# Shadylukin/Neumann

Measured on AMD Instinct MI355X. Metric: queries/sec, brute-force SIMILAR TOP-K (recall@K = 1.0 vs CPU oracle), higher is better.
Workload: dtype f32

## Files before the change

neumann_amd/csrc/nmn_api.hip:

```cpp
#include <algorithm>
#include <atomic>
#include <chrono>
#include <thread>
#include <cmath>
#include <cstdio>
#include <cstdlib>
#include <cstring>
#include <mutex>
#include <new>
#include <string>
#include <unordered_map>
#include <vector>

#include "nmn_index.h"

using namespace nmn;

namespace nmn {
float synth_value_host(uint64_t seed, uint64_t row, uint32_t col);
}

static thread_local std::string g_last_error;

static nmn_status fail_hip(hipError_t e, const char* what) {
// ... 177 lines not shown
static nmn_status ws_alloc_core(nmn_index* idx, Workspace* w);
static nmn_status ws_get(nmn_index* idx, hipStream_t stream, uint32_t nq, uint32_t k, Workspace** out) {
    Workspace* w = nullptr;
    auto it = idx->ws.find(stream);
    if (it != idx->ws.end()) w = it->second;
    uint32_t nqc = std::min(pass_queries(idx, nq), idx->ws_nq_limit);
    uint32_t cand_cap = std::max<uint32_t>(std::min<uint32_t>(idx->cand_cap, NMN_MAX_TOP_K), std::min<uint32_t>(k, NMN_MAX_TOP_K));
    if (w && w->nq_cap >= nqc && w->cand_cap >= cand_cap) {
        *out = w;
        return NMN_OK;
    }
    if (w) {
        HIP_TRY(hipStreamSynchronize(stream));
        nqc = std::max(nqc, w->nq_cap);
        cand_cap = std::max(cand_cap, w->cand_cap);
        if (w->allocated && w->cand_cap >= cand_cap) {
            Workspace* wn = new (std::nothrow) Workspace();
            if (!wn) return fail_arg(NMN_ERR_OUT_OF_MEMORY, "workspace alloc");
            wn->stream = stream;
            wn->nq_cap = nqc;
            wn->cand_cap = cand_cap;
            const nmn_status st = ws_alloc_core(idx, wn);
            if (st == NMN_OK) {
                wn->allocated = true;
                idx->ws.erase(stream);
                ws_free(w);
                idx->ws[stream] = wn;
                *out = wn;
                return NMN_OK;
            }
            ws_free(wn);
            if (st != NMN_ERR_OUT_OF_MEMORY) return st;
            idx->ws_nq_limit = std::min(idx->ws_nq_limit, w->nq_cap);
            *out = w;
            return NMN_OK;
        }
        idx->ws.erase(stream);
        ws_free(w);
    }
    w = new (std::nothrow) Workspace();
    if (!w) return fail_arg(NMN_ERR_OUT_OF_MEMORY, "workspace alloc");
    w->stream = stream;
    w->nq_cap = nqc;
    w->cand_cap = cand_cap;
    idx->ws[stream] = w;
    *out = w;
    return NMN_OK;
}

constexpr uint64_t kCrowdMinRows = 1ull << 18;
constexpr uint64_t kCrowdPool = 8ull << 20;

static void ws_release_core(Workspace* w) {
    void** ptrs[] = {(void**)&w->scores, (void**)&w->tmax, (void**)&w->wmax, (void**)&w->tsample, (void**)&w->skip_key,
                     (void**)&w->k_extra, (void**)&w->qpad, (void**)&w->qi8, (void**)&w->qinfo, (void**)&w->qinfo_f32, (void**)&w->qstate,
                     (void**)&w->cand_rows, (void**)&w->cand_scores, (void**)&w->split_sg, (void**)&w->split_ctr, (void**)&w->final_ticket, (void**)&w->done_ctr, (void**)&w->run_slots, (void**)&w->run_bound, (void**)&w->h_counts2, (void**)&w->crowd_ctr,
                     (void**)&w->crowd_rows, (void**)&w->crowd_scores, (void**)&w->fb_hist, (void**)&w->fb_list, (void**)&w->fb_count,
                     (void**)&w->fb_sync};
    for (void** p : ptrs) {
        if (*p) (void)hipFree(*p);
        *p = nullptr;
    }
    w->crowd_cap = 0;
    for (auto& e : w->ev) {
        if (e) (void)hipEventDestroy(e);
        e = nullptr;
    }
    for (auto& e : w->hist) {
        if (e) (void)hipEventDestroy(e);
        e = nullptr;
    }
    w->hist_head = w->hist_read = 0;
    w->allocated = false;
}

static nmn_status ws_alloc_core(nmn_index* idx, Workspace* w) {
    w->ld = idx->ld;
    w->score_stride = idx->cap_pad;
    w->n_tiles_cap = (uint32_t)(idx->cap_pad / kTileRows);
    const size_t nq = w->nq_cap;
    {
        static const long test_max_nq = [] { const char* e = getenv("NMN_WS_TEST_MAX_NQ"); return e ? atol(e) : 0l; }();
        if (test_max_nq > 0 && (long)nq > test_max_nq) return fail_hip(hipErrorOutOfMemory, "workspace (NMN_WS_TEST_MAX_NQ)");
    }
    HIP_TRY(hipMalloc(reinterpret_cast<void**>(&w->scores), std::max<size_t>(nq * w->score_stride, 64) * 4));
    w->tmax_stride = ((uint64_t)w->n_tiles_cap + 3) & ~3ull;
    HIP_TRY(hipMalloc(reinterpret_cast<void**>(&w->tmax), std::max<size_t>(nq * w->tmax_stride, 4) * 4));
    HIP_TRY(hipMalloc(reinterpret_cast<void**>(&w->wmax), nq * kMaxScanWaves * 4));
    w->n_sample_cap = (w->n_tiles_cap + kSampleStep - 1) / kSampleStep + 4;
    HIP_TRY(hipMalloc(reinterpret_cast<void**>(&w->tsample), nq * w->n_sample_cap * 4));
    HIP_TRY(hipMalloc(reinterpret_cast<void**>(&w->skip_key), nq * 4));
    HIP_TRY(hipMalloc(reinterpret_cast<void**>(&w->k_extra), 4));
    HIP_TRY(hipMalloc(reinterpret_cast<void**>(&w->qpad), nq * w->ld * sizeof(float)));
    HIP_TRY(hipMalloc(reinterpret_cast<void**>(&w->qi8), nq * w->ld * 2));
    HIP_TRY(hipMalloc(reinterpret_cast<void**>(&w->qinfo), nq * sizeof(QInfo)));
    HIP_TRY(hipMalloc(reinterpret_cast<void**>(&w->qinfo_f32), nq * sizeof(QInfo)));
    HIP_TRY(hipMalloc(reinterpret_cast<void**>(&w->qstate), nq * sizeof(QState)));
    HIP_TRY(hipMalloc(reinterpret_cast<void**>(&w->cand_rows), nq * w->cand_cap * sizeof(uint32_t)));
    HIP_TRY(hipMalloc(reinterpret_cast<void**>(&w->cand_scores), nq * w->cand_cap * sizeof(float)));
    {
        const size_t nqs = std::min<size_t>(nq, 4);
        HIP_TRY(hipMalloc(reinterpret_cast<void**>(&w->split_sg), nqs * 1024 * 4));
        HIP_TRY(hipMemset(w->split_sg, 0, nqs * 1024 * 4));
        HIP_TRY(hipMalloc(reinterpret_cast<void**>(&w->split_ctr), nqs * 16));
        HIP_TRY(hipMemset(w->split_ctr, 0, nqs * 16));
    }
    HIP_TRY(hipMalloc(reinterpret_cast<void**>(&w->final_ticket), nq * 4));
    HIP_TRY(hipMalloc(reinterpret_cast<void**>(&w->done_ctr), 4));
    HIP_TRY(hipMemset(w->done_ctr, 0, 4));
    HIP_TRY(hipMalloc(reinterpret_cast<void**>(&w->run_slots), nq * 1024 * 4));
    HIP_TRY(hipMalloc(reinterpret_cast<void**>(&w->run_bound), ((nq + 127) & ~(size_t)127) * 4 + 512));
    HIP_TRY(hipMemset(w->run_bound, 0, ((nq + 127) & ~(size_t)127) * 4 + 512));
    HIP_TRY(hipMemset(w->final_ticket, 0, nq * 4));
    HIP_TRY(hipMalloc(reinterpret_cast<void**>(&w->h_counts2), 2 * sizeof(unsigned long long)));
    if (idx->cap_pad >= kCrowdMinRows) {
        w->crowd_cap = (uint32_t)std::min<uint64_t>(std::max<uint64_t>(kCrowdPool, (uint64_t)nq << 17),
                                                    std::max<uint64_t>(idx->cap_pad, (uint64_t)nq * (idx->cap_pad / 8)));
        HIP_TRY(hipMalloc(reinterpret_cast<void**>(&w->crowd_ctr), (3 + (size_t)kCrowdMaxGrid) * nq * 4));
        HIP_TRY(hipMemset(w->crowd_ctr, 0, (3 + (size_t)kCrowdMaxGrid) * nq * 4));
        HIP_TRY(hipMalloc(reinterpret_cast<void**>(&w->crowd_rows), (size_t)w->crowd_cap * 4));
        HIP_TRY(hipMalloc(reinterpret_cast<void**>(&w->crowd_scores), (size_t)w->crowd_cap * 4));
        HIP_TRY(hipMalloc(reinterpret_cast<void**>(&w->fb_hist), (6 * 2048 + 2) * 4));
        HIP_TRY(hipMalloc(reinterpret_cast<void**>(&w->fb_list), nq * (size_t)NMN_MAX_TOP_K * 8));
        HIP_TRY(hipMalloc(reinterpret_cast<void**>(&w->fb_count), nq * 4));
        HIP_TRY(hipMalloc(reinterpret_cast<void**>(&w->fb_sync), 16));
        HIP_TRY(hipMemset(w->fb_sync, 0, 16));
    }
    for (auto& e : w->ev) HIP_TRY(hipEventCreate(&e));
    return NMN_OK;
}

static nmn_status ws_alloc(nmn_index* idx, Workspace* w) {
    if (w->allocated) return NMN_OK;
    for (;;) {
        const nmn_status st = ws_alloc_core(idx, w);
        if (st == NMN_OK) break;
        const std::string keep = g_last_error;
        ws_release_core(w);
        g_last_error = keep;
        if (st != NMN_ERR_OUT_OF_MEMORY || w->nq_cap <= 1) return st;
        w->nq_cap = std::max<uint32_t>(1, w->nq_cap / 4);
// ... 666 lines not shown
            sp.i8_scale = idx->q8_scale;
            sp.i8_vv = idx->q8_vv;
            sp.i8_cos = idx->q8_cos;
            sp.qi8 = w->qi8;
            sp.norms = idx->norms;
            sp.inv_norms = idx->inv_norms;
            sp.qpad = w->qpad;
            sp.qinfo = w->qinfo;
            sp.mask = mask_dev;
            sp.qmasks = qmasks_dev ? qmasks_dev + qa : nullptr;
            sp.scores = w->scores;
            sp.tmax = w->tmax;
            sp.wmax = w->wmax;
            sp.tmax_stride = w->tmax_stride;
            sp.wmax_stride = kMaxScanWaves;
            sp.n_rows = n_rows;
            sp.nql = nqc;
            sp.ld = idx->ld;
            sp.n_tiles = n_tiles;
            sp.nq = nqc;
            static const uint32_t wave_target = [] {
                const char* e = getenv("NMN_SCAN_WAVES");
                long v = e ? atol(e) : (long)kMaxScanWaves;
                return (uint32_t)std::min<long>(std::max<long>(v, 256), (long)kMaxScanWaves);
            }();
            sp.tiles_per_wave = std::max<uint32_t>(1, (n_tiles + wave_target - 1) / wave_target);
            static const bool waves_pinned = getenv("NMN_SCAN_WAVES") != nullptr;
            static const uint32_t small_waves = [] {
                const char* e = getenv("NMN_SCAN_WAVES_SMALL");
                const long v = e ? atol(e) : 768;
                return v <= 0 ? 0u : (uint32_t)std::min<long>(std::max<long>(v, 256), (long)kMaxScanWaves);
            }();
            {
                const uint64_t sweep_bytes = (uint64_t)n_rows * idx->ld * w->last_elem_bytes;
                if (!waves_pinned && small_waves && !use_mfma && !mask_dev && sweep_bytes >= (128ull << 20) && sweep_bytes < (2ull << 30))
                    sp.tiles_per_wave = std::max<uint32_t>(1, (n_tiles + small_waves - 1) / small_waves);
            }
            static const uint32_t mfma_wgs = [] {
                const char* e = getenv("NMN_MFMA_WGS");
                long v = e ? atol(e) : 1024;
                return (uint32_t)std::min<long>(std::max<long>(v, 64), (long)kMaxScanWaves);
            }();
            if (use_mfma) sp.tiles_per_wave = std::max<uint32_t>(1, (n_tiles + mfma_wgs - 1) / mfma_wgs);
            auto launch_batch_sweep = [&](const ScanParams& x) -> hipError_t { return launch_scan_mfma(x, stream); };
            static const bool no_ring = getenv("NMN_NO_RING") != nullptr;
            const bool use_ring = !no_ring && !use_mfma && !use_i8 && !use_half && nqc == 1 && !mask_dev && !qmasks_dev && n_tiles >= 4096u &&
                                  metric != NMN_METRIC_SPARSE_COSINE_F64 && scan_ring_supported(idx->ld, idx->dim, (int)metric);
            static const uint32_t ring_wgs = [] {
                const char* e = getenv("NMN_RING_WGS");
                long v = e ? atol(e) : (long)kMaxScanWaves;
                return (uint32_t)std::min<long>(std::max<long>(v, 64), (long)kMaxScanWaves);
            }();
            if (use_ring) sp.tiles_per_wave = std::max<uint32_t>(1, (n_tiles + ring_wgs - 1) / ring_wgs);
            sp.metric = (int)metric;
            sp.strided = (!use_mfma && mask_dev) ? 1u : 0u;
            static const bool no_walk = getenv("NMN_NO_WALK") != nullptr;
            sp.walk = (sp.strided && !no_walk) ? 1u : 0u;
            sp.tile_step = 1;
            sp.skip_key = nullptr;
            static const uint32_t sample_step = [] {
                const char* e = getenv("NMN_SAMPLE_STEP");
                const long v = e ? atol(e) : 0;
                return (v == 64 || v == 128 || v == 256) ? (uint32_t)v : kSampleStep;
            }();
            static const bool sample_behind = getenv("NMN_SAMPLE_AHEAD_OF_CHAIN") == nullptr;
            const uint32_t n_sample = (n_tiles + sample_step - 1) / sample_step;
            static const uint32_t run_dbg = [] { const char* e = getenv("NMN_RUN_BOUND_DEBUG"); return e ? (uint32_t)atol(e) : 0u; }();
            const bool sample = use_mfma && (!run_bound || (run_dbg & 1u)) && n_sample >= 4u * k && n_sample >= 1024u && !no_sample();
            if (run_bound) {
                sp.run_slots = w->run_slots;
                sp.run_bound = w->run_bound;
                sp.run_S = run_S;
                sp.run_dbg = run_dbg;
            }
            auto sampling_pass = [&]() -> nmn_status {
                ScanParams ss = sp;
                ss.run_S = 0;
                ss.tile_step = sample_step;
                ss.n_tiles = n_sample;
                ss.tiles_per_wave = std::max<uint32_t>(1, (n_sample + 255) / 256);
                ss.tmax = w->tsample;
                ss.tmax_stride = w->n_sample_cap;
                static const bool reread_env = getenv("NMN_SAMPLE_REREAD") != nullptr;
                const bool reread = reread_env || use_i8;
                if (!reread) {
                    ss.tmax_main = w->tmax;
                    ss.tmax_main_stride = w->tmax_stride;
                }
                HIP_TRY(launch_batch_sweep(ss));
                HIP_TRY(launch_sample_bound(w->tsample, w->n_sample_cap, n_sample, w->qinfo, nqc, k, w->skip_key, stream));
                sp.skip_key = w->skip_key;
                sp.skip_sampled = reread ? 0u : sample_step;
                return NMN_OK;
            };
            if (sample && !sample_behind) {
                st = sampling_pass();
                if (st != NMN_OK) return st;
            }
            static const bool no_chain = getenv("NMN_NO_SWEEP_CHAIN") != nullptr;
            const bool chain = !no_chain && (uint64_t)n_rows * idx->ld * w->last_elem_bytes >= (2ull << 30);
            if (chain && idx->sweep_seq && idx->sweep_stream != stream)
                HIP_TRY(hipStreamWaitEvent(stream, idx->sweep_ev[(idx->sweep_seq - 1) & 3u], 0));
            if (w->timed && qa == 0 && !nested) {
                hipEvent_t& h = w->hist[2 * (w->hist_head % Workspace::kTimingHistory)];
                if (!h) HIP_TRY(hipEventCreate(&h));
                HIP_TRY(hipEventRecord(h, stream));
            }
            if (sample && sample_behind) {
                st = sampling_pass();
                if (st != NMN_OK) return st;
            }
            static const bool no_refine = getenv("NMN_NO_REFINE") != nullptr;
            const uint32_t mfma_blocks = use_mfma ? (n_tiles + sp.tiles_per_wave - 1) / sp.tiles_per_wave : 0;
            static const uint32_t n_cu = [] {
                int dev = 0, n = 256;
                if (hipGetDevice(&dev) != hipSuccess || hipDeviceGetAttribute(&n, hipDeviceAttributeMultiprocessorCount, dev) != hipSuccess || n <= 0) n = 256;
                return (uint32_t)n;
            }();
            const uint32_t first_blocks = mfma_blocks >= 3u * n_cu ? (n_cu & ~7u) : 0u;
            static const uint32_t refine_min_nq = [] {
                const char* e = getenv("NMN_REFINE_MIN_NQ");
                return e ? (uint32_t)atol(e) : 65u;
            }();
            const uint32_t refine_from = ((use_i8 || mfma_f32) && !getenv("NMN_REFINE_MIN_NQ")) ? 3u : refine_min_nq;
            const bool refine = use_mfma && sample && nqc >= refine_from && !no_refine && first_blocks >= 64 && (uint64_t)first_blocks * sp.tiles_per_wave >= 4ull * k;
            if (qa == 0) {
                w->last_sweep_kind = use_mfma ? (use_i8 ? NMN_SWEEP_MFMA_I8 : use_half ? NMN_SWEEP_MFMA_BF16 : NMN_SWEEP_MFMA_F32)
                                              : use_i8 ? NMN_SWEEP_VALU_I8 : use_ring ? NMN_SWEEP_RING_F32 : use_half ? NMN_SWEEP_VALU_BF16 : NMN_SWEEP_VALU_F32;
                w->last_sweep_launches = (sample ? 2u : 0u) + (refine ? 3u : 1u);
            }
            if (refine) {
                ScanParams sa = sp;
                sa.bx_base = 0;
                sa.bx_count = first_blocks;
                HIP_TRY(launch_batch_sweep(sa));
                HIP_TRY(launch_sample_bound(w->tmax, w->tmax_stride, first_blocks * sp.tiles_per_wave, w->qinfo, nqc, k, w->skip_key, stream, 1));
                ScanParams sb = sp;
                sb.bx_base = first_blocks;
                sb.bx_count = 0;
                HIP_TRY(launch_batch_sweep(sb));
            } else {
                HIP_TRY(use_mfma ? launch_batch_sweep(sp) : use_i8 ? launch_scan_i8(sp, stream) : use_ring ? launch_scan_ring(sp, stream) : launch_scan(sp, stream));
            }
            if (w->timed && qa == 0 && !nested) {
                hipEvent_t& h = w->hist[2 * (w->hist_head % Workspace::kTimingHistory) + 1];
                if (!h) HIP_TRY(hipEventCreate(&h));
                HIP_TRY(hipEventRecord(h, stream));
                w->hist_head++;
                w->scan_ev_in_hist = true;
            }
            if (chain) {
                hipEvent_t& ce = idx->sweep_ev[idx->sweep_seq & 3u];
                if (!ce) HIP_TRY(hipEventCreateWithFlags(&ce, hipEventDisableTiming));
// ... 848 lines not shown
    *calls_per_s = (double)calls.load() / dt;
    if (merged_batches) *merged_batches = b1 - b0;
    if (merged_calls) *merged_calls = r1 - r0;
    if (mismatches) *mismatches = bad.load();
    return NMN_OK;
}

extern "C" nmn_status nmn_index_coalesce_stats(nmn_index* idx, uint64_t* batches, uint64_t* requests) {
    if (!idx) return fail_arg(NMN_ERR_INVALID_ARGUMENT, "null index");
    std::lock_guard<std::mutex> g(idx->mu);
    if (batches) *batches = idx->coalesced_batches;
    if (requests) *requests = idx->coalesced_requests;
    return NMN_OK;
}

extern "C" nmn_status nmn_index_search(nmn_index* idx, const float* queries, uint32_t nq, uint32_t k,
                                       nmn_metric metric, const uint64_t* mask, uint64_t* out_rows,
                                       float* out_scores, uint32_t* out_counts, nmn_search_stats* stats) {
    const nmn_status st = index_search_hostio(idx, queries, nq, k, (int)metric, mask, false, out_rows, out_scores, out_counts, stats);
    if (st == NMN_OK && stats && mask && stats->rows_scanned && idx->dim) {
        const uint64_t n = stats->rows_scanned, eb = stats->bytes_scanned / (n * idx->dim);
        uint64_t kept = 0;
        for (uint64_t wd = 0; wd < n / 64; wd++) kept += (uint64_t)__builtin_popcountll(mask[wd]);
        if (n % 64) kept += (uint64_t)__builtin_popcountll(mask[n / 64] & ((1ull << (n % 64)) - 1));
        stats->rows_scanned = kept;
        stats->bytes_scanned = kept * idx->dim * eb;
    }
    return st;
}

extern "C" nmn_status nmn_index_search_dmask(nmn_index* idx, const float* queries, uint32_t nq, uint32_t k,
                                             nmn_metric metric, const uint64_t* mask_dev, uint64_t* out_rows,
                                             float* out_scores, uint32_t* out_counts, nmn_search_stats* stats) {
    return index_search_hostio(idx, queries, nq, k, (int)metric, mask_dev, true, out_rows, out_scores, out_counts, stats);
}

extern "C" nmn_status nmn_index_search_dmask_hint(nmn_index* idx, const float* queries, uint32_t nq, uint32_t k,
                                                  nmn_metric metric, const uint64_t* mask_dev, uint64_t mask_rows,
                                                  uint64_t* out_rows, float* out_scores, uint32_t* out_counts,
                                                  nmn_search_stats* stats) {
    return index_search_hostio(idx, queries, nq, k, (int)metric, mask_dev, true, out_rows, out_scores, out_counts, stats,
                               mask_rows);
}

extern "C" nmn_status nmn_index_read_probe(nmn_index* idx, uint32_t reps, double* gbps_out) {
    if (!idx || !gbps_out) return fail_arg(NMN_ERR_INVALID_ARGUMENT, "null argument");
    *gbps_out = 0.0;
    if (idx->rows == 0) return NMN_OK;
    HIP_TRY(hipSetDevice(idx->device));
    std::unique_lock<std::mutex> lk(idx->mu);
    IdleGuard idle(idx, lk);
    hipStream_t s = idx->host_stream;
    float* sink = nullptr;
    HIP_TRY(hipMalloc(reinterpret_cast<void**>(&sink), 4));
    hipEvent_t a = nullptr, b = nullptr;
    hipError_t e = hipEventCreate(&a);
    if (e == hipSuccess) e = hipEventCreate(&b);
    float best = 0.f;
    const uint64_t n_tiles = idx->rows / kTileRows;
    const bool ring = n_tiles >= 4096u && scan_ring_supported(idx->ld, idx->dim, NMN_METRIC_DOT_PRODUCT) && !getenv("NMN_NO_RING");
    const uint32_t ring_tpw = (uint32_t)std::max<uint64_t>(1, (n_tiles + kMaxScanWaves - 1) / kMaxScanWaves);
    uint64_t probe_rows = ring ? n_tiles * kTileRows : idx->rows;
    auto probe = [&]() { return ring ? launch_ring_probe(idx->corpus, idx->rows, idx->ld, ring_tpw, s) : launch_read_probe(idx->corpus, idx->rows, idx->ld, sink, s); };
    if (e == hipSuccess) e = probe();
    for (uint32_t i = 0; i < std::max(reps, 1u) && e == hipSuccess; i++) {
        e = hipEventRecord(a, s);
        if (e == hipSuccess) e = probe();
        if (e == hipSuccess) e = hipEventRecord(b, s);
        if (e == hipSuccess) e = hipEventSynchronize(b);
        float ms = 0.f;
        if (e == hipSuccess) e = hipEventElapsedTime(&ms, a, b);
        if (e == hipSuccess && ms > 0.f && (best == 0.f || ms < best)) best = ms;
    }
    if (a) (void)hipEventDestroy(a);
    if (b) (void)hipEventDestroy(b);
    (void)hipFree(sink);
    if (e != hipSuccess) return fail_hip(e, "nmn_index_read_probe");
    if (best > 0.f) *gbps_out = (double)probe_rows * idx->ld * 4.0 / (best * 1e-3) / 1e9;
    return NMN_OK;
}

extern "C" nmn_status nmn_index_score_rows(nmn_index* idx, const float* queries, uint32_t nq, nmn_metric metric,
                                           const uint64_t* local_rows, uint32_t n_rows, float* out_scores) {
    if (!idx || !queries || !local_rows || !out_scores) return fail_arg(NMN_ERR_INVALID_ARGUMENT, "null argument");
    if (nq == 0 || n_rows == 0) return NMN_OK;
    if (nq > NMN_MAX_QUERIES) return fail_arg(NMN_ERR_INVALID_ARGUMENT, "nq out of range");
    for (uint32_t i = 0; i < n_rows; i++)
        if (local_rows[i] >= idx->rows) return fail_arg(NMN_ERR_NOT_FOUND, "row out of range");
    HIP_TRY(hipSetDevice(idx->device));
    std::unique_lock<std::mutex> lk(idx->mu);
    IdleGuard idle(idx, lk);
    hipStream_t s = idx->host_stream;
    float *dq = nullptr, *dqpad = nullptr, *dout = nullptr;
    QInfo* dqi = nullptr;
    QState* dqs = nullptr;
    uint64_t* drows = nullptr;
    auto done = [&](nmn_status st) {
        for (void* p : {(void*)dq, (void*)dqpad, (void*)dout, (void*)dqi, (void*)dqs, (void*)drows})
            if (p) (void)hipFree(p);
        return st;
    };
    hipError_t e;
#define TRY2(x) if ((e = (x)) != hipSuccess) return done(fail_hip(e, #x))
    TRY2(hipMalloc(reinterpret_cast<void**>(&dq), (size_t)nq * idx->dim * 4));
    TRY2(hipMalloc(reinterpret_cast<void**>(&dqpad), (size_t)nq * idx->ld * 4));
    TRY2(hipMalloc(reinterpret_cast<void**>(&dout), (size_t)nq * n_rows * 4));
    TRY2(hipMalloc(reinterpret_cast<void**>(&dqi), (size_t)nq * sizeof(QInfo)));
    TRY2(hipMalloc(reinterpret_cast<void**>(&dqs), (size_t)nq * sizeof(QState)));
    TRY2(hipMalloc(reinterpret_cast<void**>(&drows), (size_t)n_rows * 8));
    TRY2(hipMemcpyAsync(dq, queries, (size_t)nq * idx->dim * 4, hipMemcpyHostToDevice, s));
    TRY2(hipMemcpyAsync(drows, local_rows, (size_t)n_rows * 8, hipMemcpyHostToDevice, s));
    TRY2(launch_qprep(dq, nq, idx->dim, idx->ld, (int)metric, idx->max_norm_bits, dqpad, dqi, dqs, 0, s));
    TRY2(launch_score_rows(idx->corpus, idx->norms, dqpad, dqi, drows, n_rows, nq, idx->ld, idx->dim, (int)metric,
                           dout, s));
    TRY2(hipMemcpyAsync(out_scores, dout, (size_t)nq * n_rows * 4, hipMemcpyDeviceToHost, s));
    TRY2(hipStreamSynchronize(s));
// ... 157 lines not shown
```

neumann_amd/csrc/nmn_index.h:

```cpp
#pragma once
#include <condition_variable>
#include <mutex>
#include <string>
#include <unordered_map>
#include <vector>

#include "nmn_internal.h"

using nmn::QInfo;
using nmn::QState;
using nmn::kDefaultCandCap;

struct Workspace {
    hipStream_t stream = nullptr;
    uint32_t nq_cap = 0;
    uint32_t cand_cap = 0;
    uint64_t score_stride = 0;
    uint32_t n_tiles_cap = 0;
    uint32_t ld = 0;
    uint32_t* scores = nullptr;
    uint32_t* tmax = nullptr;
    uint32_t* wmax = nullptr;
    uint32_t* tsample = nullptr;
    uint32_t* skip_key = nullptr;
    uint32_t* k_extra = nullptr;
    uint32_t* crowd_ctr = nullptr;
    uint32_t* crowd_rows = nullptr;
    float* crowd_scores = nullptr;
    uint32_t crowd_cap = 0;
    uint32_t* fb_hist = nullptr;
    unsigned long long* fb_list = nullptr;
    uint32_t* fb_count = nullptr;
    unsigned long long* fb_sync = nullptr;
    uint64_t n_sample_cap = 0;
    uint64_t tmax_stride = 0;
    float* qpad = nullptr;
    uint32_t* qi8 = nullptr;
    QInfo* qinfo = nullptr;
    QInfo* qinfo_f32 = nullptr;
    QState* qstate = nullptr;
    uint32_t* cand_rows = nullptr;
    float* cand_scores = nullptr;
    uint32_t* run_slots = nullptr;
    uint32_t* run_bound = nullptr;
    uint32_t* split_sg = nullptr;
    uint32_t* split_ctr = nullptr;
    uint32_t* final_ticket = nullptr;
    float* h_queries = nullptr;  size_t h_queries_cap = 0;
    uint64_t* h_mask = nullptr;  size_t h_mask_cap = 0;
    uint64_t* h_out_rows = nullptr; float* h_out_scores = nullptr; uint32_t* h_out_counts = nullptr;
    size_t h_out_rows_cap = 0, h_out_scores_cap = 0, h_cnt_cap = 0;
    uint8_t* h_pack = nullptr; size_t h_pack_cap = 0;
    const uint64_t** h_qmasks = nullptr; size_t h_qmasks_cap = 0;
    uint8_t* pred_block = nullptr; size_t pred_block_cap = 0;
    uint64_t* pred_masks = nullptr; size_t pred_masks_cap = 0;
    uint32_t* pred_ticket = nullptr; size_t pred_ticket_cap = 0;
    unsigned long long* pred_counts = nullptr; size_t pred_counts_cap = 0;
    uint8_t* pin_pred = nullptr; size_t pin_pred_cap = 0;
    uint8_t* pin_in = nullptr; size_t pin_in_cap = 0;
    uint8_t* pin_out = nullptr; size_t pin_out_cap = 0;
    uint32_t done_seq = 0;
    uint32_t* done_ctr = nullptr;
    uint32_t* poll_word_dev = nullptr;
    uint8_t* pin_in_dev = nullptr;
    uint8_t* pin_out_dev = nullptr;
    unsigned long long* tiny_pool = nullptr;
    uint32_t* tiny_ticket = nullptr;
    uint8_t* tiny_out = nullptr;
    uint8_t* tiny_out_dev = nullptr;
    uint32_t tiny_seq = 0;
    uint64_t* h_rowlist = nullptr; size_t h_rowlist_cap = 0;
    float* h_scorelist = nullptr; size_t h_scorelist_cap = 0;
    unsigned long long* h_counts2 = nullptr;
    uint64_t* lk_keys = nullptr; size_t lk_keys_cap = 0;
    hipEvent_t ev[4] = {nullptr, nullptr, nullptr, nullptr};
// ... 141 lines not shown
```

neumann_amd/csrc/nmn_internal.h:

```cpp
#pragma once
#include <hip/hip_runtime.h>
#include <stdint.h>

#include "../../include/neumann_gpu.h"

namespace nmn {

constexpr int kMetricNegL2 = 16;
constexpr int kMetricNegL2Sq = 17;

constexpr uint32_t kTileRows = 64;
constexpr uint32_t kDefaultCandCap = 4096;
constexpr uint32_t kMaxScanWaves = 4096;
constexpr uint32_t kKeyMasked = 0u;
constexpr uint32_t kKeyNaN = 1u;
constexpr uint32_t kScoreSentinelBits = 0xFFFFFFFFu;

struct QInfo {
    float qmag;
    float margin_abs;
    float margin_rel;
    float pad;
    float qscale;
    float qq8;
// ... 65 lines not shown
        if (thr == thr) {
            Tc = score_to_key(thr);
            if (Tc > T) Tc = T;
            if (Tc < kKeyNaN) Tc = kKeyNaN;
        }
    }
    return Tc;
}


__host__ __device__ inline uint64_t score_at(uint64_t row, uint32_t q, uint32_t nql) {
    return ((row >> 6) * nql + q) * 64ull + (row & 63ull);
}

struct ScanParams {
    const float* corpus;
    const float* corpus_half;
    const int8_t* corpus_i8;
    const float* i8_scale;
    const float* i8_vv;
    const float* i8_cos;
    const uint32_t* qi8;
    const QState* retry_state;
    const float* norms;
    const float* inv_norms;
    const float* qpad;
    const QInfo* qinfo;
    const uint64_t* mask;
    const uint64_t* const* qmasks;
    uint32_t* scores;
    uint32_t* tmax;
    uint32_t* wmax;
    uint64_t tmax_stride;
    uint64_t wmax_stride;
    uint64_t n_rows;
    uint32_t nql;
    uint32_t tile_step;
    uint32_t fold_ny;
    const uint32_t* skip_key;
    uint32_t* tmax_main;
    uint64_t tmax_main_stride;
    uint32_t skip_sampled;
    uint32_t ld;
    uint32_t n_tiles;
    uint32_t nq;
    uint32_t tiles_per_wave;
    uint32_t strided;
    uint32_t walk;
    uint32_t bx_base, bx_count;
    uint32_t* run_slots;
    uint32_t* run_bound;
    uint32_t run_S;
    uint32_t i8_one_plane;
    uint32_t run_dbg;
    int metric;
};
hipError_t launch_scan(const ScanParams& p, hipStream_t s);
bool scan_ring_supported(uint32_t ld, uint32_t dim, int metric);
hipError_t launch_scan_ring(const ScanParams& p, hipStream_t s);
hipError_t launch_half_rows(const float* corpus, float* half, uint32_t ld, uint64_t row0, uint64_t n, const float* norms,
                            float* row_err2_scratch, uint32_t* err_bits, hipStream_t s);
bool scan_half_supported(uint32_t ld, int metric);
bool scan_i8_supported(uint32_t ld, uint32_t dim, int metric);
hipError_t launch_scan_i8(const ScanParams& p, hipStream_t s);
hipError_t launch_q8_rows(const float* corpus, int8_t* q8, float* scale, float* vv, float* cosf, uint32_t ld, uint64_t row0, uint64_t n, const float* norms,
                          float* row_err2_scratch, uint32_t* err_bits, hipStream_t s);
bool ingest_supported(uint32_t ld, uint32_t dim);
bool exact_rows_supported(uint32_t ld, uint32_t dim, int metric);
hipError_t launch_exact_rows(const float* corpus, const float* norms, uint32_t ld, uint64_t n_rows, const float* qpad, const QInfo* qinfo,
                             const QState* qstate, int flagged, const uint64_t* mask, const uint64_t* const* qmasks, uint32_t* scores,
                             uint32_t nql, uint32_t nq, int metric, hipStream_t s);
hipError_t launch_ingest(const float* corpus, uint32_t ld, uint64_t row0, uint64_t n, float* norms, float* inv_norms,
                         uint32_t* max_norm_bits, float* half, uint32_t* err_bits, hipStream_t s);
bool ingest_q8_supported(uint32_t ld, uint32_t dim);
hipError_t launch_ingest_q8(const float* corpus, uint32_t ld, uint64_t row0, uint64_t n, float* norms, float* inv_norms, uint32_t* max_norm_bits,
                            int8_t* q8, float* scale, float* vv, float* cosf, uint32_t* err_bits, hipStream_t s);
hipError_t launch_read_probe(const float* corpus, uint64_t n_rows, uint32_t ld, float* sink, hipStream_t s);
hipError_t launch_ring_probe(const float* corpus, uint64_t n_rows, uint32_t ld, uint32_t tiles_per_wg, hipStream_t s);
bool scan_mfma_supported(uint32_t ld, uint32_t dim, int metric);
hipError_t launch_scan_mfma(const ScanParams& p, hipStream_t s);
hipError_t launch_scan_mfma_f32(const ScanParams& p, hipStream_t s);
bool scan_mfma_i8_supported(uint32_t ld, uint32_t dim, int metric);
bool scan_mfma_i8_one_plane_supported(int metric);
hipError_t launch_scan_mfma_i8_one(const ScanParams& p, hipStream_t s);

struct SelectParams {
    const uint32_t* scores;
    const uint32_t* tmax;
    const uint32_t* wmax;
    uint64_t tmax_stride;
    uint64_t wmax_stride;
    uint32_t n_waves;
    uint32_t tiles_per_wave;
    uint32_t strided;
    const QInfo* qinfo;
    QState* qstate;
    uint32_t* cand_rows;
    uint64_t n_rows;
    uint32_t nql;
    uint32_t n_tiles;
    uint32_t nq;
    uint32_t k;
    uint32_t cand_cap;
    const uint32_t* skip_key;
    const uint32_t* k_extra;
    int retry;
    uint32_t* half_stats;
    int retry_follows;
    unsigned long long* fb_sync_reset;
    uint32_t* crowd_count_reset;
    int crowd_follows;
    float* l2_hint;
    int count_overflows;
    int flat;
    uint32_t split;
    uint32_t* split_sg;
    uint32_t* split_ctr;
};
hipError_t launch_select(const SelectParams& p, hipStream_t s);
hipError_t launch_count_untrusted(const float* norms, uint64_t n_rows, uint32_t* out, hipStream_t s);
hipError_t launch_sample_bound(const uint32_t* tmax_sample, uint64_t stride, uint32_t n_sample, const QInfo* qinfo,
                               uint32_t nq, uint32_t k, uint32_t* skip_key, hipStream_t s, int combine_max = 0);

struct CrowdParams {
    QState* qstate;
    const uint32_t* tmax;
    uint64_t tmax_stride;
    const uint32_t* scores;
    uint32_t nql, nq, n_tiles;
    uint64_t n_rows;
    uint32_t* count;
// ... 140 lines not shown
```

neumann_amd/csrc/nmn_scan_ring.hip:

```cpp
#include <algorithm>
#include <cstdlib>

#include "nmn_internal.h"

namespace nmn {

namespace {

typedef float f4 __attribute__((ext_vector_type(4)));
typedef uint32_t u4 __attribute__((ext_vector_type(4)));

constexpr int kRingStageBytes = 64 * 128 * 4;
constexpr int kRingStages = 4;
constexpr int kRingPieces = 8;
constexpr int kRingRowPitch = 128;

template <int N>
__device__ __forceinline__ void ring_wait_vm() {
    asm volatile("s_waitcnt vmcnt(%0)" ::"n"(N) : "memory");
}

template <int METRIC, bool PROBE = false>
__global__ void __launch_bounds__(256, 1) scan_ring_kernel(ScanParams p) {
    extern __shared__ __attribute__((aligned(16))) float lds[];
    float* const nrm = lds + kRingStages * (kRingStageBytes / 4);
    uint32_t* const tpart = reinterpret_cast<uint32_t*>(nrm + 8 * 64);
    float* const qlds = nrm + 8 * 64 + 8;
    const uint32_t KC = p.ld / 128u;
    constexpr bool kL2 = METRIC == NMN_METRIC_EUCLIDEAN;
    constexpr bool kCos = METRIC == NMN_METRIC_COSINE;
    const uint32_t lane = threadIdx.x & 63u;
    const uint32_t wave = __builtin_amdgcn_readfirstlane(threadIdx.x >> 6);
    const uint32_t r4 = lane >> 4, j = lane & 15u;
    const uint32_t ld = p.ld;
    const uint32_t row_bytes = ld * 4u;
    const uint32_t bx = blockIdx.x;
    const uint32_t t0 = bx * p.tiles_per_wave;
    if (t0 >= p.n_tiles) return;
    const uint32_t t1 = min(t0 + p.tiles_per_wave, p.n_tiles);
    const uint32_t n_stage = (t1 - t0) * KC;

    for (uint32_t c = wave; !PROBE && c * 256u < ld; c += 4u) {
        if (c * 256u + lane * 4u < ld)
            __builtin_amdgcn_global_load_lds((const __attribute__((address_space(1))) void*)(p.qpad + c * 256u + lane * 4u),
                                             (__attribute__((address_space(3))) void*)(qlds + c * 256u), 16, 0, 0);
    }
    const float qmag = PROBE ? 1.f : p.qinfo[0].qmag;

    uint32_t loff[kRingPieces];
#pragma unroll
    for (int pp = 0; pp < kRingPieces; pp++) {
        const uint32_t r = 2u * (wave * kRingPieces + (uint32_t)pp) + lane / 32u;
        loff[pp] = r * row_bytes + (((lane % 32u) ^ (r & 15u)) * 16u);
    }
    const char* const mat = reinterpret_cast<const char*>(p.corpus);
    auto stage_src = [&](uint32_t tile_, uint32_t kc_) -> const char* {
        return mat + (uint64_t)tile_ * kTileRows * row_bytes + (uint64_t)kc_ * 512u;
    };
    auto issue_stage = [&](const char* src, uint32_t lmask, uint32_t slot) __attribute__((always_inline)) {
#pragma unroll
        for (int pp = 0; pp < kRingPieces; pp++)
            __builtin_amdgcn_global_load_lds((const __attribute__((address_space(1))) void*)(src + (loff[pp] & lmask)),
                                             (__attribute__((address_space(3))) void*)(lds + slot * (kRingStageBytes / 4) +
                                                                                        (wave * kRingPieces + (uint32_t)pp) * 256u),
                                             16, 0, 2);
    };
    auto norms_dma = [&](uint32_t tile_, uint32_t rel) __attribute__((always_inline)) {
        __builtin_amdgcn_global_load_lds((const __attribute__((address_space(1))) void*)(p.norms + (uint64_t)tile_ * kTileRows + lane),
                                         (__attribute__((address_space(3))) void*)(nrm + (rel & 7u) * 64u), 4, 0, 0);
    };
#pragma unroll
    for (uint32_t s0 = 0; s0 < kRingStages; s0++) {
        if (s0 < n_stage) {
            if (!PROBE && kCos && wave == 0 && s0 % KC == 0) norms_dma(t0 + s0 / KC, s0 / KC);
            if (s0 < kRingStages - 1) issue_stage(stage_src(t0 + s0 / KC, s0 % KC), 0xFFFFFFFFu, s0 % kRingStages);
        } else if (s0 < kRingStages - 1) {
            issue_stage(mat, 0u, s0 % kRingStages);
        }
    }
    constexpr int kSub = 4;
    uint32_t off[kSub];
#pragma unroll
    for (int sub = 0; sub < kSub; sub++) {
        const uint32_t rr = (uint32_t)sub * 4u + r4;
        off[sub] = (wave * 16u + rr) * kRingRowPitch + (((j * 2u) ^ rr) * 4u);
    }

    uint32_t wmax = kKeyMasked;
    uint32_t sidx = 0;
    uint32_t nt = t0 + (kRingStages - 1) / KC, nkc = (kRingStages - 1) % KC;
    for (uint32_t tile = t0; tile < t1; tile++) {
        float acc[kSub][2];
#pragma unroll
        for (int sub = 0; sub < kSub; sub++) acc[sub][0] = acc[sub][1] = 0.f;
        for (uint32_t kc = 0; kc < KC; kc++, sidx++) {
            const float* buf = lds + (sidx % kRingStages) * (kRingStageBytes / 4);
            ring_wait_vm<(kRingStages - 2) * kRingPieces>();
            if (kc == 0) __builtin_amdgcn_s_barrier();
            asm volatile("" ::: "memory");
            if (!PROBE && kc == 0 && wave == 0 && tile > t0) {
                const uint32_t* tp = tpart + ((tile - 1u - t0) & 1u) * 4u;
                const uint32_t m = max(max(tp[0], tp[1]), max(tp[2], tp[3]));
                if (lane == 0) p.tmax[tile - 1u] = m;
                wmax = max(wmax, m);
            }
            const uint32_t ns = sidx + (kRingStages - 1);
            const bool issue = ns < n_stage;
            const char* const nsrc = issue ? stage_src(nt, nkc) : mat;
            const uint32_t lmask = issue ? 0xFFFFFFFFu : 0u;
            float* const nbuf = lds + (ns % kRingStages) * (kRingStageBytes / 4);
            f4 a[kSub][2];
            f4 q0 = {0.f, 0.f, 0.f, 0.f}, q1 = q0;
            if constexpr (!PROBE) {
#pragma unroll
                for (int sub = 0; sub < kSub; sub++) {
                    a[sub][0] = *reinterpret_cast<const f4*>(buf + off[sub]);
                    a[sub][1] = *reinterpret_cast<const f4*>(buf + (off[sub] ^ 4u));
                }
                q0 = *reinterpret_cast<const f4*>(qlds + kc * 128u + j * 8u);
                q1 = *reinterpret_cast<const f4*>(qlds + kc * 128u + j * 8u + 4u);
            }
#pragma unroll
            for (int sub = 0; sub < kSub; sub++) {
#pragma unroll
                for (int pp = sub * 2; pp < sub * 2 + 2; pp++)
                    __builtin_amdgcn_global_load_lds((const __attribute__((address_space(1))) void*)(nsrc + (loff[pp] & lmask)),
                                                     (__attribute__((address_space(3))) void*)(nbuf + (wave * kRingPieces + (uint32_t)pp) * 256u), 16, 0, 2);
                if constexpr (PROBE) continue;
                const f4 x0 = a[sub][0], x1 = a[sub][1];
                if constexpr (kL2) {
                    const f4 d0 = x0 - q0, d1 = x1 - q1;
#pragma unroll
                    for (int e = 0; e < 4; e++) {
                        acc[sub][0] = __builtin_fmaf(d0[e], d0[e], acc[sub][0]);
                        acc[sub][1] = __builtin_fmaf(d1[e], d1[e], acc[sub][1]);
                    }
                } else {
#pragma unroll
                    for (int e = 0; e < 4; e++) {
                        acc[sub][0] = __builtin_fmaf(x0[e], q0[e], acc[sub][0]);
                        acc[sub][1] = __builtin_fmaf(x1[e], q1[e], acc[sub][1]);
                    }
                }
            }
            asm volatile("s_waitcnt lgkmcnt(0)" ::: "memory");
            if (++nkc == KC) {
                nkc = 0;
                nt++;
            }
            if (!PROBE && kCos && wave == 0 && ns + 1u < n_stage && nkc == 0) norms_dma(nt, nt - t0);
        }
        if constexpr (PROBE) continue;
        float v = 0.f;
#pragma unroll
        for (int sub = 0; sub < kSub; sub++) {
            float t = acc[sub][0] + acc[sub][1];
            t += __int_as_float(__builtin_amdgcn_update_dpp(0, __float_as_int(t), 0x128, 0xF, 0xF, false));
            t += __int_as_float(__builtin_amdgcn_update_dpp(0, __float_as_int(t), 0x124, 0xF, 0xF, false));
            t += __int_as_float(__builtin_amdgcn_update_dpp(0, __float_as_int(t), 0x122, 0xF, 0xF, false));
            t += __int_as_float(__builtin_amdgcn_update_dpp(0, __float_as_int(t), 0x121, 0xF, 0xF, false));
            if ((j & 3u) == (uint32_t)sub) v = t;
        }
        const uint32_t wrow = (j & 3u) * 4u + r4;
        const uint64_t row = (uint64_t)tile * kTileRows + wave * 16u + wrow;
        const bool valid = row < p.n_rows;
        float sc;
        if constexpr (kCos) {
            const float vn = nrm[((tile - t0) & 7u) * 64u + wave * 16u + wrow];
            sc = (vn == 0.f || qmag == 0.f) ? 0.f : v / (qmag * vn);
        } else if constexpr (kL2) {
            const float dist = sqrtf(fmaxf(v, 0.f));
            sc = p.metric == kMetricNegL2 ? -dist : 1.0f / (1.0f + dist);
        } else {
            sc = v;
        }
        uint32_t key = valid ? score_to_key(sc) : kKeyMasked;
        if (j < 4u) p.scores[row] = valid ? f2u(sc) : kScoreSentinelBits;
#pragma unroll
        for (int o = 1; o < 64; o <<= 1) key = max(key, (uint32_t)__shfl_xor((int)key, o));
        if (lane == 0) tpart[((tile - t0) & 1u) * 4u + wave] = key;
        asm volatile("s_waitcnt lgkmcnt(0)" ::: "memory");
    }
    ring_wait_vm<0>();
    __builtin_amdgcn_s_barrier();
    asm volatile("" ::: "memory");
    if (!PROBE && wave == 0) {
        const uint32_t* tp = tpart + ((t1 - 1u - t0) & 1u) * 4u;
        const uint32_t m = max(max(tp[0], tp[1]), max(tp[2], tp[3]));
        wmax = max(wmax, m);
        if (lane == 0) {
            p.tmax[t1 - 1u] = m;
            p.wmax[bx] = wmax;
        }
    }
}

template <int METRIC>
hipError_t launch_ring_metric(const ScanParams& p, hipStream_t s) {
    const uint32_t blocks = (p.n_tiles + p.tiles_per_wave - 1) / p.tiles_per_wave;
    const size_t lds = (size_t)kRingStages * kRingStageBytes + 8 * 64 * 4 + 8 * 4 + (size_t)p.ld * 4;
    auto kern = scan_ring_kernel<METRIC>;
    hipError_t e = hipFuncSetAttribute(reinterpret_cast<const void*>(kern), hipFuncAttributeMaxDynamicSharedMemorySize, (int)lds);
    if (e != hipSuccess) return e;
    hipLaunchKernelGGL(kern, dim3(blocks), dim3(256), lds, s, p);
    return hipGetLastError();
}

}

bool scan_ring_supported(uint32_t ld, uint32_t dim, int metric) {
    if (!(metric == NMN_METRIC_COSINE || metric == NMN_METRIC_DOT_PRODUCT || metric == NMN_METRIC_EUCLIDEAN || metric == kMetricNegL2)) return false;
    return dim <= ld && ld % 128u == 0 && ld >= 128u && ld <= 4096u;
}

hipError_t launch_ring_probe(const float* corpus, uint64_t n_rows, uint32_t ld, uint32_t tiles_per_wg, hipStream_t s) {
    ScanParams p{};
    p.corpus = corpus;
    p.n_rows = n_rows;
    p.ld = ld;
    p.n_tiles = (uint32_t)(n_rows / kTileRows);
    p.tiles_per_wave = std::max<uint32_t>(1, tiles_per_wg);
    if (p.n_tiles == 0) return hipSuccess;
    const uint32_t blocks = (p.n_tiles + p.tiles_per_wave - 1) / p.tiles_per_wave;
    const size_t lds = (size_t)kRingStages * kRingStageBytes + 8 * 64 * 4 + 8 * 4 + (size_t)p.ld * 4;
    auto kern = scan_ring_kernel<NMN_METRIC_DOT_PRODUCT, true>;
    hipError_t e = hipFuncSetAttribute(reinterpret_cast<const void*>(kern), hipFuncAttributeMaxDynamicSharedMemorySize, (int)lds);
    if (e != hipSuccess) return e;
    hipLaunchKernelGGL(kern, dim3(blocks), dim3(256), lds, s, p);
    return hipGetLastError();
}

hipError_t launch_scan_ring(const ScanParams& p, hipStream_t s) {
    switch (p.metric) {
        case NMN_METRIC_COSINE: return launch_ring_metric<NMN_METRIC_COSINE>(p, s);
        case NMN_METRIC_EUCLIDEAN:
        case kMetricNegL2: return launch_ring_metric<NMN_METRIC_EUCLIDEAN>(p, s);
        default: return launch_ring_metric<NMN_METRIC_DOT_PRODUCT>(p, s);
    }
}

}
```

Before: 220.9.

## Use persistent ring-scan workgroups with atomic ticket scheduling and weighted tail chunks

The ring scan kernel now launches one workgroup per CU, and each workgroup pulls chunk tickets from a global atomic counter instead of owning a single fixed tile range. Chunks are sized unevenly: main chunks are larger and a set of smaller tail chunks comes last, which is meant to balance load and shorten the straggler tail of the full-corpus sweep. Per-group wmax values are flushed with plain stores or atomicMax when a chunk spans group boundaries, wmax is zeroed before each launch, and the counters reset themselves at the end of the kernel. In exchange this adds atomics and extra barriers per chunk, and it relies on the counter reset being correct across launches.

```diff
diff --git a/neumann_amd/csrc/nmn_api.hip b/neumann_amd/csrc/nmn_api.hip
--- a/neumann_amd/csrc/nmn_api.hip
+++ b/neumann_amd/csrc/nmn_api.hip
@@ -253,7 +253,7 @@
 constexpr uint64_t kCrowdPool = 8ull << 20;
 
 static void ws_release_core(Workspace* w) {
-    void** ptrs[] = {(void**)&w->scores, (void**)&w->tmax, (void**)&w->wmax, (void**)&w->tsample, (void**)&w->skip_key,
+    void** ptrs[] = {(void**)&w->scores, (void**)&w->tmax, (void**)&w->wmax, (void**)&w->ring_ctr, (void**)&w->tsample, (void**)&w->skip_key,
                      (void**)&w->k_extra, (void**)&w->qpad, (void**)&w->qi8, (void**)&w->qinfo, (void**)&w->qinfo_f32, (void**)&w->qstate,
                      (void**)&w->cand_rows, (void**)&w->cand_scores, (void**)&w->split_sg, (void**)&w->split_ctr, (void**)&w->final_ticket, (void**)&w->done_ctr, (void**)&w->run_slots, (void**)&w->run_bound, (void**)&w->h_counts2, (void**)&w->crowd_ctr,
                      (void**)&w->crowd_rows, (void**)&w->crowd_scores, (void**)&w->fb_hist, (void**)&w->fb_list, (void**)&w->fb_count,
@@ -288,6 +288,8 @@
     w->tmax_stride = ((uint64_t)w->n_tiles_cap + 3) & ~3ull;
     HIP_TRY(hipMalloc(reinterpret_cast<void**>(&w->tmax), std::max<size_t>(nq * w->tmax_stride, 4) * 4));
     HIP_TRY(hipMalloc(reinterpret_cast<void**>(&w->wmax), nq * kMaxScanWaves * 4));
+    HIP_TRY(hipMalloc(reinterpret_cast<void**>(&w->ring_ctr), 2 * 4));
+    HIP_TRY(hipMemset(w->ring_ctr, 0, 2 * 4));
     w->n_sample_cap = (w->n_tiles_cap + kSampleStep - 1) / kSampleStep + 4;
     HIP_TRY(hipMalloc(reinterpret_cast<void**>(&w->tsample), nq * w->n_sample_cap * 4));
     HIP_TRY(hipMalloc(reinterpret_cast<void**>(&w->skip_key), nq * 4));
@@ -1060,6 +1062,7 @@
                 return (uint32_t)std::min<long>(std::max<long>(v, 64), (long)kMaxScanWaves);
             }();
             if (use_ring) sp.tiles_per_wave = std::max<uint32_t>(1, (n_tiles + ring_wgs - 1) / ring_wgs);
+            ring_set_grid(sp, use_ring ? w->ring_ctr : nullptr);
             sp.metric = (int)metric;
             sp.strided = (!use_mfma && mask_dev) ? 1u : 0u;
             static const bool no_walk = getenv("NMN_NO_WALK") != nullptr;
@@ -1107,6 +1110,7 @@
             }
             static const bool no_chain = getenv("NMN_NO_SWEEP_CHAIN") != nullptr;
             const bool chain = !no_chain && (uint64_t)n_rows * idx->ld * w->last_elem_bytes >= (2ull << 30);
+            if (sp.ring_wgs) HIP_TRY(hipMemsetAsync(w->wmax, 0, (size_t)((n_tiles + sp.tiles_per_wave - 1) / sp.tiles_per_wave) * sizeof(uint32_t), stream));
             if (chain && idx->sweep_seq && idx->sweep_stream != stream)
                 HIP_TRY(hipStreamWaitEvent(stream, idx->sweep_ev[(idx->sweep_seq - 1) & 3u], 0));
             if (w->timed && qa == 0 && !nested) {
@@ -2061,7 +2065,8 @@
     IdleGuard idle(idx, lk);
     hipStream_t s = idx->host_stream;
     float* sink = nullptr;
-    HIP_TRY(hipMalloc(reinterpret_cast<void**>(&sink), 4));
+    HIP_TRY(hipMalloc(reinterpret_cast<void**>(&sink), 2 * 4));
+    HIP_TRY(hipMemset(sink, 0, 2 * 4));
     hipEvent_t a = nullptr, b = nullptr;
     hipError_t e = hipEventCreate(&a);
     if (e == hipSuccess) e = hipEventCreate(&b);
@@ -2070,7 +2075,7 @@
     const bool ring = n_tiles >= 4096u && scan_ring_supported(idx->ld, idx->dim, NMN_METRIC_DOT_PRODUCT) && !getenv("NMN_NO_RING");
     const uint32_t ring_tpw = (uint32_t)std::max<uint64_t>(1, (n_tiles + kMaxScanWaves - 1) / kMaxScanWaves);
     uint64_t probe_rows = ring ? n_tiles * kTileRows : idx->rows;
-    auto probe = [&]() { return ring ? launch_ring_probe(idx->corpus, idx->rows, idx->ld, ring_tpw, s) : launch_read_probe(idx->corpus, idx->rows, idx->ld, sink, s); };
+    auto probe = [&]() { return ring ? launch_ring_probe(idx->corpus, idx->rows, idx->ld, ring_tpw, reinterpret_cast<uint32_t*>(sink), s) : launch_read_probe(idx->corpus, idx->rows, idx->ld, sink, s); };
     if (e == hipSuccess) e = probe();
     for (uint32_t i = 0; i < std::max(reps, 1u) && e == hipSuccess; i++) {
         e = hipEventRecord(a, s);
diff --git a/neumann_amd/csrc/nmn_index.h b/neumann_amd/csrc/nmn_index.h
--- a/neumann_amd/csrc/nmn_index.h
+++ b/neumann_amd/csrc/nmn_index.h
@@ -21,6 +21,7 @@
     uint32_t* scores = nullptr;
     uint32_t* tmax = nullptr;
     uint32_t* wmax = nullptr;
+    uint32_t* ring_ctr = nullptr;
     uint32_t* tsample = nullptr;
     uint32_t* skip_key = nullptr;
     uint32_t* k_extra = nullptr;
diff --git a/neumann_amd/csrc/nmn_internal.h b/neumann_amd/csrc/nmn_internal.h
--- a/neumann_amd/csrc/nmn_internal.h
+++ b/neumann_amd/csrc/nmn_internal.h
@@ -141,6 +141,10 @@
     uint32_t* run_bound;
     uint32_t run_S;
     uint32_t i8_one_plane;
+    uint32_t ring_wgs;
+    uint32_t ring_tail;
+    uint32_t ring_grid;
+    uint32_t* ring_ctr;
     uint32_t run_dbg;
     int metric;
 };
@@ -165,7 +169,8 @@
 hipError_t launch_ingest_q8(const float* corpus, uint32_t ld, uint64_t row0, uint64_t n, float* norms, float* inv_norms, uint32_t* max_norm_bits,
                             int8_t* q8, float* scale, float* vv, float* cosf, uint32_t* err_bits, hipStream_t s);
 hipError_t launch_read_probe(const float* corpus, uint64_t n_rows, uint32_t ld, float* sink, hipStream_t s);
-hipError_t launch_ring_probe(const float* corpus, uint64_t n_rows, uint32_t ld, uint32_t tiles_per_wg, hipStream_t s);
+hipError_t launch_ring_probe(const float* corpus, uint64_t n_rows, uint32_t ld, uint32_t tiles_per_wg, uint32_t* ctr, hipStream_t s);
+void ring_set_grid(ScanParams& p, uint32_t* ctr);
 bool scan_mfma_supported(uint32_t ld, uint32_t dim, int metric);
 hipError_t launch_scan_mfma(const ScanParams& p, hipStream_t s);
 hipError_t launch_scan_mfma_f32(const ScanParams& p, hipStream_t s);
diff --git a/neumann_amd/csrc/nmn_scan_ring.hip b/neumann_amd/csrc/nmn_scan_ring.hip
--- a/neumann_amd/csrc/nmn_scan_ring.hip
+++ b/neumann_amd/csrc/nmn_scan_ring.hip
@@ -14,6 +14,14 @@
 constexpr int kRingStages = 4;
 constexpr int kRingPieces = 8;
 constexpr int kRingRowPitch = 128;
+constexpr uint32_t kRingTailWeight = 4;
+
+#ifdef NMN_RING_WG_CLOCK
+__device__ unsigned long long* nmn_ring_clk;
+#define NMN_RING_CLK(i, v) do { if (threadIdx.x == 0) nmn_ring_clk[(uint64_t)blockIdx.x * 5u + (i)] = (v); } while (0)
+#else
+#define NMN_RING_CLK(i, v) do { } while (0)
+#endif
 
 template <int N>
 __device__ __forceinline__ void ring_wait_vm() {
@@ -34,10 +42,29 @@
     const uint32_t r4 = lane >> 4, j = lane & 15u;
     const uint32_t ld = p.ld;
     const uint32_t row_bytes = ld * 4u;
-    const uint32_t bx = blockIdx.x;
-    const uint32_t t0 = bx * p.tiles_per_wave;
-    if (t0 >= p.n_tiles) return;
-    const uint32_t t1 = min(t0 + p.tiles_per_wave, p.n_tiles);
+    NMN_RING_CLK(0, wall_clock64());
+    NMN_RING_CLK(4, __smid());
+    const uint32_t tpw = p.tiles_per_wave;
+    auto first_tile = [&](uint32_t b) -> uint32_t {
+        const uint64_t gm = p.ring_wgs - p.ring_tail;
+        const uint64_t u = b <= gm ? (uint64_t)kRingTailWeight * b : (uint64_t)kRingTailWeight * gm + (b - gm);
+        return (uint32_t)(u * p.n_tiles / ((uint64_t)kRingTailWeight * gm + p.ring_tail));
+    };
+    uint32_t* const ticket = reinterpret_cast<uint32_t*>(qlds + ld);
+    for (uint32_t round = 0;; round++) {
+    uint32_t bx = blockIdx.x;
+    if (p.ring_wgs) {
+        if (threadIdx.x == 0) *ticket = atomicAdd(p.ring_ctr, 1u);
+        __syncthreads();
+        bx = __builtin_amdgcn_readfirstlane(*ticket);
+        __syncthreads();
+        if (bx >= p.ring_wgs) break;
+    } else if (round) {
+        break;
+    }
+    const uint32_t t0 = p.ring_wgs ? first_tile(bx) : bx * tpw;
+    const uint32_t t1 = p.ring_wgs ? first_tile(bx + 1u) : min(t0 + tpw, p.n_tiles);
+    if (t0 >= p.n_tiles || t1 <= t0) continue;
     const uint32_t n_stage = (t1 - t0) * KC;
 
     for (uint32_t c = wave; !PROBE && c * 256u < ld; c += 4u) {
@@ -87,6 +114,11 @@
     }
 
     uint32_t wmax = kKeyMasked;
+    auto flush_group = [&](uint32_t g, uint32_t m) __attribute__((always_inline)) {
+        if (lane != 0) return;
+        if (g * tpw >= t0 && min(g * tpw + tpw, p.n_tiles) <= t1) p.wmax[g] = m;
+        else atomicMax(p.wmax + g, m);
+    };
     uint32_t sidx = 0;
     uint32_t nt = t0 + (kRingStages - 1) / KC, nkc = (kRingStages - 1) % KC;
     for (uint32_t tile = t0; tile < t1; tile++) {
@@ -98,14 +130,20 @@
             ring_wait_vm<(kRingStages - 2) * kRingPieces>();
             if (kc == 0) __builtin_amdgcn_s_barrier();
             asm volatile("" ::: "memory");
+            if (sidx == 0) NMN_RING_CLK(1, wall_clock64());
             if (!PROBE && kc == 0 && wave == 0 && tile > t0) {
                 const uint32_t* tp = tpart + ((tile - 1u - t0) & 1u) * 4u;
                 const uint32_t m = max(max(tp[0], tp[1]), max(tp[2], tp[3]));
                 if (lane == 0) p.tmax[tile - 1u] = m;
                 wmax = max(wmax, m);
+                if (tile % tpw == 0) {
+                    flush_group((tile - 1u) / tpw, wmax);
+                    wmax = kKeyMasked;
+                }
             }
             const uint32_t ns = sidx + (kRingStages - 1);
             const bool issue = ns < n_stage;
+            if (ns == n_stage) NMN_RING_CLK(2, wall_clock64());
             const char* const nsrc = issue ? stage_src(nt, nkc) : mat;
             const uint32_t lmask = issue ? 0xFFFFFFFFu : 0u;
             float* const nbuf = lds + (ns % kRingStages) * (kRingStageBytes / 4);
@@ -188,17 +226,21 @@
         const uint32_t* tp = tpart + ((t1 - 1u - t0) & 1u) * 4u;
         const uint32_t m = max(max(tp[0], tp[1]), max(tp[2], tp[3]));
         wmax = max(wmax, m);
-        if (lane == 0) {
-            p.tmax[t1 - 1u] = m;
-            p.wmax[bx] = wmax;
-        }
-    }
+        if (lane == 0) p.tmax[t1 - 1u] = m;
+        flush_group((t1 - 1u) / tpw, wmax);
+    }
+    }
+    if (p.ring_wgs && threadIdx.x == 0 && atomicAdd(p.ring_ctr + 1, 1u) == gridDim.x - 1u) {
+        p.ring_ctr[0] = 0u;
+        p.ring_ctr[1] = 0u;
+    }
+    NMN_RING_CLK(3, wall_clock64());
 }
 
 template <int METRIC>
 hipError_t launch_ring_metric(const ScanParams& p, hipStream_t s) {
-    const uint32_t blocks = (p.n_tiles + p.tiles_per_wave - 1) / p.tiles_per_wave;
-    const size_t lds = (size_t)kRingStages * kRingStageBytes + 8 * 64 * 4 + 8 * 4 + (size_t)p.ld * 4;
+    const uint32_t blocks = p.ring_wgs ? p.ring_grid : (p.n_tiles + p.tiles_per_wave - 1) / p.tiles_per_wave;
+    const size_t lds = (size_t)kRingStages * kRingStageBytes + 8 * 64 * 4 + 8 * 4 + (size_t)p.ld * 4 + 16;
     auto kern = scan_ring_kernel<METRIC>;
     hipError_t e = hipFuncSetAttribute(reinterpret_cast<const void*>(kern), hipFuncAttributeMaxDynamicSharedMemorySize, (int)lds);
     if (e != hipSuccess) return e;
@@ -213,16 +255,38 @@
     return dim <= ld && ld % 128u == 0 && ld >= 128u && ld <= 4096u;
 }
 
-hipError_t launch_ring_probe(const float* corpus, uint64_t n_rows, uint32_t ld, uint32_t tiles_per_wg, hipStream_t s) {
+void ring_set_grid(ScanParams& p, uint32_t* ctr) {
+    struct Grid {
+        uint32_t chunks, tail, wgs;
+    };
+    static const Grid g = []() -> Grid {
+        if (getenv("NMN_NO_RING_EVEN")) return {0, 0, 0};
+        int dev = 0, n = 256;
+        if (hipGetDevice(&dev) != hipSuccess || hipDeviceGetAttribute(&n, hipDeviceAttributeMultiprocessorCount, dev) != hipSuccess || n <= 0) n = 256;
+        auto knob = [](const char* name, long def) {
+            const char* e = getenv(name);
+            return std::min<long>(std::max<long>(e ? atol(e) : def, 0), 32);
+        };
+        const long m = std::max<long>(knob("NMN_RING_MAIN", 14), 1), t = knob("NMN_RING_TAIL", 8);
+        return {(uint32_t)((m + t) * n), (uint32_t)(t * n), (uint32_t)n};
+    }();
+    p.ring_wgs = ctr ? g.chunks : 0u;
+    p.ring_tail = g.tail;
+    p.ring_grid = g.wgs;
+    p.ring_ctr = ctr;
+}
+
+hipError_t launch_ring_probe(const float* corpus, uint64_t n_rows, uint32_t ld, uint32_t tiles_per_wg, uint32_t* ctr, hipStream_t s) {
     ScanParams p{};
     p.corpus = corpus;
     p.n_rows = n_rows;
     p.ld = ld;
     p.n_tiles = (uint32_t)(n_rows / kTileRows);
     p.tiles_per_wave = std::max<uint32_t>(1, tiles_per_wg);
+    ring_set_grid(p, ctr);
     if (p.n_tiles == 0) return hipSuccess;
-    const uint32_t blocks = (p.n_tiles + p.tiles_per_wave - 1) / p.tiles_per_wave;
-    const size_t lds = (size_t)kRingStages * kRingStageBytes + 8 * 64 * 4 + 8 * 4 + (size_t)p.ld * 4;
+    const uint32_t blocks = p.ring_wgs ? p.ring_grid : (p.n_tiles + p.tiles_per_wave - 1) / p.tiles_per_wave;
+    const size_t lds = (size_t)kRingStages * kRingStageBytes + 8 * 64 * 4 + 8 * 4 + (size_t)p.ld * 4 + 16;
     auto kern = scan_ring_kernel<NMN_METRIC_DOT_PRODUCT, true>;
     hipError_t e = hipFuncSetAttribute(reinterpret_cast<const void*>(kern), hipFuncAttributeMaxDynamicSharedMemorySize, (int)lds);
     if (e != hipSuccess) return e;
```

Result: faster. 225.7 (median of 6 runs) (+2.2%).
